# BjarkeHautop/bayesSSM

Measured on AMD Instinct MI355X. Metric: particle-steps/sec (N x T), bootstrap filter, higher is better.
Workload: dtype f64; 1 GPU; BASELINE C2: linear-Gaussian SSM, bootstrap filter, T=1000, N=1048576, SISR + systematic resampling, return_particles=FALSE, device generator; per_gpu=one independent filter replica per GPU (no data-path collective), backend=single process

## Files before the change

### bayesssm_amd/csrc/fused.hip.h

```cpp
#pragma once
#include "kernels.hip.h"

namespace bssm {

typedef unsigned long long fz_u64;
#define BSSM_RLX_AGENT __ATOMIC_RELAXED, __HIP_MEMORY_SCOPE_AGENT

constexpr int FZ_MAXB = 2 * NT;
constexpr int FZ_MINB = 256;
constexpr int FZ_KREC = 8;
constexpr int FZ_KSIDE = (int)(sizeof(SideEntry) / 4);
constexpr int FZ_NREP = 16;
constexpr int FZ_MAXSIDE = 16;
constexpr uint32_t FLAG_FUSED_BAIL = 8u, FLAG_FUSED_TIMEOUT = 16u;
constexpr uint32_t FZ_ST_DOIT = 1u, FZ_ST_DEAD = 2u, FZ_ST_STOP = 4u, FZ_ST_BAIL = 8u;
constexpr long long FZ_TIMEOUT_TICKS = 2000000ll;

struct FusedWs {
    fz_u64 e1[6][FZ_MAXB];
    fz_u64 c1[FZ_NREP][16];
    fz_u64 m1[FZ_NREP][16];
    fz_u64 a1[2][FZ_MAXB];
    fz_u64 e2[FZ_KREC][FZ_MAXB];
    fz_u64 c2[FZ_NREP][16];
    fz_u64 e3[FZ_KREC][FZ_MAXB];
    fz_u64 c3[FZ_NREP][16];
    fz_u64 a3[2][FZ_MAXB];
    fz_u64 side_w[FZ_MAXB][FZ_MAXSIDE][FZ_KSIDE];
    fz_u64 side_p[FZ_MAXB][FZ_MAXSIDE][FZ_KSIDE];
    BlockRec brec_priv[2][MAXB];
    SideList side_priv[2][FZ_MAXB];
    long long stamps[2][24];
    long long startt[FZ_MAXB];
    long long endt[FZ_MAXB];
    long long waket[4][FZ_MAXB];
    long long pubt[4][FZ_MAXB];
};

#ifdef BSSM_DEV_STAMPS
#define FZ_STAMP(k) do { if (fz_stamper) g.ws->stamps[fz_row][k] = clock64(); } while (0)
#else
#define FZ_STAMP(k) do { } while (0)
#endif

__device__ __forceinline__ fz_u64 fz_gran(uint32_t tag, uint32_t v) { return ((fz_u64)tag << 32) | v; }
__device__ __forceinline__ void fz_put(fz_u64* g, uint32_t tag, uint32_t v) { __hip_atomic_store(g, fz_gran(tag, v), BSSM_RLX_AGENT); }
__device__ __forceinline__ void fz_put64(fz_u64* g, uint32_t tag, uint64_t v) { fz_put(g, tag, (uint32_t)v); fz_put(g + 1, tag, (uint32_t)(v >> 32)); }
__device__ __forceinline__ void fz_put64x(fz_u64* g, int stride, uint32_t tag, uint64_t v) { fz_put(g, tag, (uint32_t)v); fz_put(g + stride, tag, (uint32_t)(v >> 32)); }
__device__ __forceinline__ fz_u64 fz_get(const fz_u64* g) { return __hip_atomic_load(g, BSSM_RLX_AGENT); }

__device__ __forceinline__ void fz_encode(const BlockRec& br, uint32_t (&w)[FZ_KREC])
{
    const Rec& r = br.prefix;
    const long long d1 = (long long)(r.o[1] - r.o[0]), d2 = (long long)(r.o[2] - r.o[0]), d3 = (long long)(r.o[3] - r.o[0]);
    const bool fits = d1 >= -32768 && d1 <= 32767 && d2 >= -32768 && d2 <= 32767 && d3 >= -32768 && d3 <= 32767;
    const uint32_t meta = (uint32_t)(r.kind & 3) | ((uint32_t)(br.nside & 127) << 2) | ((br.tail_from < NT) ? (1u << 9) : 0u) | (fits ? 0u : (1u << 10));
    w[0] = (uint32_t)r.base; w[1] = (uint32_t)(r.base >> 32); w[2] = (uint32_t)r.o[0]; w[3] = (uint32_t)(r.o[0] >> 32);
    w[4] = ((uint32_t)d1 & 0xffffu) | (((uint32_t)d2 & 0xffffu) << 16);
    w[5] = ((uint32_t)d3 & 0xffffu) | (meta << 16);
    w[6] = (uint32_t)r.lo; w[7] = (uint32_t)r.hi;
}
__device__ __forceinline__ BlockRec fz_decode(const uint32_t (&w)[FZ_KREC], bool& unsupported)
{
    BlockRec br;
    Rec& r = br.prefix;
    r.base = mk64(w[0], w[1]); r.o[0] = mk64(w[2], w[3]);
    r.o[1] = r.o[0] + (uint64_t)(long long)(int16_t)(w[4] & 0xffffu);
    r.o[2] = r.o[0] + (uint64_t)(long long)(int16_t)(w[4] >> 16);
    r.o[3] = r.o[0] + (uint64_t)(long long)(int16_t)(w[5] & 0xffffu);
    const uint32_t meta = w[5] >> 16;
    r.kind = (int32_t)(meta & 3); r.lo = (int32_t)w[6]; r.hi = (int32_t)w[7]; r.pad = 0;
    br.nside = (int32_t)((meta >> 2) & 127);
    const bool tail = (meta >> 9) & 1u, unenc = (meta >> 10) & 1u;
    br.tail_from = tail ? 0 : NT;
    unsupported = tail || unenc || br.nside > FZ_MAXSIDE;
    return br;
}

struct FzClock { long long t0; __device__ __forceinline__ bool expired() const { return (long long)wall_clock64() - t0 > FZ_TIMEOUT_TICKS; } };

template <int NG>
__device__ __forceinline__ bool fz_wait_slot(const fz_u64* slot, uint32_t tag, const FzClock& clk, uint32_t& val)
{
    const int lane = threadIdx.x & 63;
    for (unsigned spins = 0;; spins++) {
        bool ok = true;
        if (lane < NG) { const fz_u64 x = fz_get(slot + lane); ok = (uint32_t)(x >> 32) == tag; val = (uint32_t)x; }
        if (__all(ok)) return true;
        if ((spins & 31u) == 31u && clk.expired()) return false;
        __builtin_amdgcn_s_sleep(1);
    }
}

template <int NG>
__device__ __forceinline__ bool fz_wait_words(const fz_u64* mine, uint32_t tag, const FzClock& clk, uint32_t& val)
{
    const int lane = threadIdx.x & 63;
    for (unsigned spins = 0;; spins++) {
        bool ok = true;
        if (lane < NG) { const fz_u64 x = fz_get(mine); ok = (uint32_t)(x >> 32) == tag; val = (uint32_t)x; }
        if (__all(ok)) return true;
        if ((spins & 31u) == 31u && clk.expired()) return false;
        __builtin_amdgcn_s_sleep(1);
    }
}

struct LaneTerms { double a[EL]; };
__device__ __attribute__((noinline)) void fz_block_literal(uint64_t* tin , uint64_t cin, double* terms , const LaneTerms v ,
                                                           DevState* st)
{
    const int t = threadIdx.x;
#pragma unroll
    for (int k = 0; k < EL; k++) terms[t * EL + k] = v.a[k];
    __syncthreads();
    if (t == 0) {
        double c = b2d(cin);
        for (int tt = 0; tt < NT; tt++) {
            tin[tt] = d2b(c);
            for (int k = 0; k < EL; k++) c = c + terms[tt * EL + k];
        }
        atomicAdd((unsigned long long*)&st->stat_serial_walks, 1ull);
        atomicAdd((unsigned long long*)&st->stat_literal_terms, (unsigned long long)EB);
    }
    __syncthreads();
}
__device__ __forceinline__ LaneTerms fz_lane_terms(const double (&v)[EL])
{
    LaneTerms r;
#pragma unroll
    for (int k = 0; k < EL; k++) r.a[k] = v[k];
    return r;
}

struct FusedRecSink {
    fz_u64* rec_planes;
    fz_u64* side_base;
    int bidx; uint32_t tag;
    double* terms; DevState* st;
    __device__ __forceinline__ void rec(const BlockRec& br) const
    {
        uint32_t w[FZ_KREC];
        fz_encode(br, w);
#pragma unroll
        for (int k = 0; k < FZ_KREC; k++) fz_put(rec_planes + (size_t)k * FZ_MAXB + bidx, tag, w[k]);
    }
    __device__ __forceinline__ void side(int k, const SideEntry& e) const
    {
        if (k >= FZ_MAXSIDE) return;
        uint32_t w[FZ_KSIDE];
        memcpy(w, &e, sizeof(SideEntry));
        fz_u64* dst = side_base + ((size_t)bidx * FZ_MAXSIDE + k) * FZ_KSIDE;
#pragma unroll
        for (int q = 0; q < FZ_KSIDE; q++) fz_put(dst + q, tag, w[q]);
    }
    __device__ __forceinline__ void literal(uint64_t* tin, uint64_t cin, const double (&v)[EL]) const { fz_block_literal(tin, cin, terms, fz_lane_terms(v), st); }
};

struct FusedArgs {
    const double* xin;
    long long N; int nblk;
    ModelPar par; double y; NoiseSrc ns; int trans;
    int obs_i, resample_algorithm; double threshold;
    double* ess_out; double* llh_out; int* resampled_out;
    double* w_out;
    int lim;
    int force_fallback;
    int early_max;
    ApplyArgs a;
    FusedWs* ws; uint32_t tag;
    double* znext; uint32_t znext_call;
};

struct FusedSmem {
    double red[16]; double redq[16];
    uint32_t slot[16];
    int bail;
    double bm, bs_, bq;
};

template <int NG>
__device__ __forceinline__ bool fz_gather(const fz_u64* planes, int c0, int c1, uint32_t tag, const FzClock& clk, int* bail, uint32_t (&w0)[NG], uint32_t (&w1)[NG])
{
    const bool pair = ((c0 & 1) == 0) && (c0 < c1);
    const bool want1 = (c0 + 1 < c1);
    __amdgpu_buffer_rsrc_t rs = __builtin_amdgcn_make_buffer_rsrc((void*)const_cast<fz_u64*>(planes), 0, NG * FZ_MAXB * 8, 0x00020000);
    bool have = false;
    for (unsigned spins = 0;; spins++) {
        if (!have) {
            bool ok = true;
            if (pair) {
#pragma unroll
                for (int k = 0; k < NG; k++) {
                    const u32x4_t x = __builtin_amdgcn_raw_buffer_load_b128(rs, (k * FZ_MAXB + c0) * 8, 0, 16);
                    ok = ok && x.y == tag && (!want1 || x.w == tag); w0[k] = x.x; w1[k] = x.z;
                }
            } else {
#pragma unroll
                for (int k = 0; k < NG; k++) {
                    if (c0 < c1) { const fz_u64 x = fz_get(planes + (size_t)k * FZ_MAXB + c0); ok = ok && (uint32_t)(x >> 32) == tag; w0[k] = (uint32_t)x; }
                    if (c0 + 1 < c1) { const fz_u64 x = fz_get(planes + (size_t)k * FZ_MAXB + c0 + 1); ok = ok && (uint32_t)(x >> 32) == tag; w1[k] = (uint32_t)x; }
                }
            }
            have = ok;
        }
        if (__all(have)) return true;
        if ((spins & 15u) == 15u && clk.expired()) { *bail = 1; return false; }
        if (*(volatile int*)bail) return false;
        __builtin_amdgcn_s_sleep(1);
    }
}

__device__ __forceinline__ bool fz_fetch_sides(const fz_u64* side_base, SideList* side_priv, int b, int nside, uint32_t tag, const FzClock& clk)
{
    for (int k = 0; k < nside; k++) {
        const fz_u64* src = side_base + ((size_t)b * FZ_MAXSIDE + k) * FZ_KSIDE;
        uint32_t w[FZ_KSIDE];
        for (unsigned spins = 0;; spins++) {
            bool ok = true;
#pragma unroll
            for (int q = 0; q < FZ_KSIDE; q++) { const fz_u64 x = fz_get(src + q); ok = ok && (uint32_t)(x >> 32) == tag; w[q] = (uint32_t)x; }
            if (ok) break;
            if ((spins & 15u) == 15u && clk.expired()) return false;
            __builtin_amdgcn_s_sleep(1);
        }
        SideEntry e;
        memcpy(&e, w, sizeof(SideEntry));
        side_priv[b].e[k] = e;
    }
    return true;
}

struct FzLateSide {
    static constexpr bool active = true;
    const fz_u64* src; uint32_t tag; FzClock clk;
    __device__ __forceinline__ unsigned long long issue() const
    {
        const int lane = threadIdx.x & 63;
        static_assert(FZ_KSIDE <= 64, "one granule per lane");
        return (lane < FZ_KSIDE) ? fz_get(src + lane) : 0ull;
    }
    __device__ __forceinline__ bool finish(SideEntry* dst, unsigned long long x) const
    {
        const int lane = threadIdx.x & 63;
        for (unsigned spins = 0;; spins++) {
            const bool ok = (lane >= FZ_KSIDE) || ((uint32_t)(x >> 32) == tag);
            if (__all(ok)) {
                if (lane < FZ_KSIDE) reinterpret_cast<uint32_t*>(dst)[lane] = (uint32_t)x;
                __builtin_amdgcn_fence(__ATOMIC_RELEASE, "wavefront");
                __builtin_amdgcn_wave_barrier();
                __builtin_amdgcn_fence(__ATOMIC_ACQUIRE, "wavefront");
                return true;
            }
            if ((spins & 15u) == 15u && clk.expired()) return false;
            __builtin_amdgcn_s_sleep(1);
            if (lane < FZ_KSIDE) x = fz_get(src + lane);
        }
    }
};

template <int MODE, bool EMIT>
__device__ __forceinline__ uint64_t fz_resolve_duty(SegSmem& sm, ResolveSmem& rs, FusedSmem& fs, const FusedArgs& g, DevState* st, const FzClock& clk,
                                                    uint64_t* cin_lds , bool& bail)
{
    const int t = threadIdx.x, B = g.nblk;
    const fz_u64* planes = (MODE == MODE_W) ? &g.ws->e2[0][0] : &g.ws->e3[0][0];
    const fz_u64* sides = (MODE == MODE_W) ? &g.ws->side_w[0][0][0] : &g.ws->side_p[0][0][0];
    const int CB = (B + NT - 1) / NT;
    const int Bneed = (MODE == MODE_P) ? B - 1 : B;
    const int c0 = t * CB, c1 = (c0 + CB < Bneed) ? c0 + CB : Bneed;
    uint32_t w0[FZ_KREC], w1[FZ_KREC];
    bool ok = fz_gather<FZ_KREC>(planes, c0, c1, g.tag, clk, &fs.bail, w0, w1);
    bool unsup = false;
    BlockRec q0, q1;
    q0.prefix = rec_identity(0); q0.tail_from = NT; q0.nside = 0; q1 = q0;
    if (ok) {
        if (c0 < c1) {
            bool u; q0 = fz_decode(w0, u); unsup = unsup || u;
            if (!u && q0.nside > 0 && !(c0 == B - 1 && q0.nside == 1 && q0.tail_from >= NT)) {
#ifdef BSSM_DEV_STAMPS
                g.ws->pubt[3][20 + MODE] = c0; atomicAdd((unsigned long long*)&g.ws->pubt[3][22 + MODE], 1ull);
#endif
                ok = ok && fz_fetch_sides(sides, g.ws->side_priv[MODE], c0, q0.nside, g.tag, clk);
            }
        }
        if (c0 + 1 < c1) {
            bool u; q1 = fz_decode(w1, u); unsup = unsup || u;
            if (!u && q1.nside > 0 && !(c0 + 1 == B - 1 && q1.nside == 1 && q1.tail_from >= NT)) {
#ifdef BSSM_DEV_STAMPS
                g.ws->pubt[3][20 + MODE] = c0 + 1; atomicAdd((unsigned long long*)&g.ws->pubt[3][22 + MODE], 1ull);
#endif
                ok = ok && fz_fetch_sides(sides, g.ws->side_priv[MODE], c0 + 1, q1.nside, g.tag, clk);
            }
        }
    }
    if (unsup) atomicMax(&fs.bail, 2); else if (!ok) atomicMax(&fs.bail, 1);
    __syncthreads();
#ifdef BSSM_DEV_STAMPS
    if (t == 0) { g.ws->stamps[1][MODE == MODE_W ? 8 : 13] = clock64(); g.ws->pubt[3][8 + (MODE == MODE_W ? 1 : 2)] = (long long)wall_clock64(); }
#endif
    if (fs.bail) { bail = true; return 0ull; }
    long long lit = 0;
    const int upto = (MODE == MODE_P) ? B - 1 : B;
    FzLateSide late; late.src = sides + ((size_t)(B - 1) * FZ_MAXSIDE + 0) * FZ_KSIDE; late.tag = g.tag; late.clk = clk;
    const uint64_t fin = resolve_in_block<MODE, NT, EMIT, FzLateSide>(sm, rs, g.ws->brec_priv[MODE], g.ws->side_priv[MODE], B, upto, g.xin, g.N, 1.0, st, true, g.force_fallback, cin_lds, &lit, &q0, &q1, late);
    if (EMIT && t == 0) cin_lds[B - 1] = fin;
    if (lit >= LIT_FROM_W) fs.bail = 2;
    __syncthreads();
#ifdef BSSM_DEV_STAMPS
    if (t == 0) g.ws->stamps[1][MODE == MODE_W ? 9 : 14] = clock64();
#endif
    if (fs.bail) { bail = true; return 0ull; }
    return fin;
}

__host__ __device__ __forceinline__ int fz_resolver_block(int B) { return (5 * B) / 16; }

__device__ __forceinline__ void fz_draw_next(const FusedArgs& g, long long j0, long long N, const int prio_after = 1)
{
    if (!g.znext) return;
    __builtin_amdgcn_s_setprio(0);
#pragma unroll
    for (int i = 0; i < EL / 2; i++) {
        const long long j = j0 + 2 * i;
        if (j < N) {
            double z0, z1;
            normal_pair(g.ns.key, g.ns.purpose, g.znext_call, 0, (uint32_t)(j >> 1), z0, z1);
            if (j + 1 < N) bulk_store16<1>(g.znext + j, z0, z1);
            else g.znext[j] = z0;
        }
    }
    if (prio_after == 3) __builtin_amdgcn_s_setprio(3); else __builtin_amdgcn_s_setprio(1);
}

template <int MODEL, int KIND>
__global__ __launch_bounds__(NT) void k_obs(FusedArgs g, DevState* st)
{
    __shared__ SegSmem sm;
    __shared__ uint64_t tin[NT + 1];
    __shared__ FusedSmem fs;
    __shared__ int Tbegin;
    extern __shared__ __attribute__((aligned(16))) double dyn[];
    int* Tl = reinterpret_cast<int*>(dyn);
    double* lx = dyn + EB / 2;
    const int t = threadIdx.x, lane = t & 63, wave = t >> 6;
    const int bidx = (int)blockIdx.x, B = g.nblk;
    const bool resolver = (bidx == fz_resolver_block(B));
    if (resolver) __builtin_amdgcn_s_setprio(3); else __builtin_amdgcn_s_setprio(1);
    const bool fz_stamper = (t == 0) && (resolver || bidx == ((B > 100) ? 100 : 0)); const int fz_row = resolver ? 1 : 0; (void)fz_stamper; (void)fz_row;
    FZ_STAMP(0);
#ifdef BSSM_DEV_STAMPS
    if (t == 0) g.ws->startt[bidx] = (long long)wall_clock64();
#define FZ_PUBT(k) do { if (t == 0) g.ws->pubt[k][bidx] = (long long)wall_clock64(); } while (0)
#define FZ_GDONE(k) do { if (t == 0) g.ws->pubt[3][8 + (k)] = (long long)wall_clock64(); } while (0)
#define FZ_WAKE(k) do { if (t == 0) g.ws->waket[k][bidx] = (long long)wall_clock64(); } while (0)
#else
#define FZ_PUBT(k) do { } while (0)
#define FZ_GDONE(k) do { } while (0)
#define FZ_WAKE(k) do { } while (0)
#endif
    const long long b0 = (long long)bidx * EB, j0 = b0 + (long long)t * EL;
    const long long N = g.N;
    FzClock clk; clk.t0 = (long long)wall_clock64();
    const int s_dead = st->dead, call = st->res_calls;
    const uint32_t s_flags = st->flags;
    if (t == 0) fs.bail = 0;
    double x8[EL], l8[EL];
    if (j0 + EL <= N) {
        const double2* p = reinterpret_cast<const double2*>(g.xin + j0);
#pragma unroll
        for (int k = 0; k < EL / 2; k++) { const double2 q = p[k]; x8[2 * k] = q.x; x8[2 * k + 1] = q.y; }
    } else {
#pragma unroll
        for (int k = 0; k < EL; k++) x8[k] = (j0 + k < N) ? g.xin[j0 + k] : 0.0;
    }
    double z8[EL];
#pragma unroll
    for (int i = 0; i < EL / 2; i++) {
        const long long j = j0 + 2 * i;
        z8[2 * i] = 0.0; z8[2 * i + 1] = 0.0;
        if (g.trans && j < N) {
            if (g.ns.arr) { if (j + 1 < N) { const double2 q = *reinterpret_cast<const double2*>(g.ns.arr + j); z8[2 * i] = q.x; z8[2 * i + 1] = q.y; } else { z8[2 * i] = g.ns.arr[j]; } }
            else normal_pair(g.ns.key, g.ns.purpose, g.ns.call, 0, (uint32_t)(j >> 1), z8[2 * i], z8[2 * i + 1]);
        }
    }
    if (s_dead || s_flags) return;
#pragma unroll
    for (int i = 0; i < EL / 2; i++) {
        const long long j = j0 + 2 * i;
        if (g.trans && j < N) {
            x8[2 * i] = Model<MODEL>::transition(x8[2 * i], z8[2 * i], g.par);
            x8[2 * i + 1] = Model<MODEL>::transition(x8[2 * i + 1], z8[2 * i + 1], g.par);
        }
        l8[2 * i] = (j < N) ? r_dnorm_log(g.y, x8[2 * i], g.par.sy, g.par.log_sy) : -INFINITY;
        l8[2 * i + 1] = (j + 1 < N) ? r_dnorm_log(g.y, x8[2 * i + 1], g.par.sy, g.par.log_sy) : -INFINITY;
    }
    FZ_STAMP(1);
    double bm;
    {
        double m = l8[0];
#pragma unroll
        for (int k = 1; k < EL; k++) m = fmax(m, l8[k]);
        m = wave_max(m);
        __syncthreads();
        if (lane == 0) fs.red[wave] = m;
        __syncthreads();
        bm = fs.red[0];
#pragma unroll
        for (int i = 1; i < NWV; i++) bm = fmax(bm, fs.red[i]);
    }
    const bool early = (g.early_max != 0);
    if (early && t < 2) { const uint64_t bits = d2b(bm); fz_put(&g.ws->e1[t][bidx], g.tag, t ? (uint32_t)(bits >> 32) : (uint32_t)bits); }
    double bsum, bsq;
    {
        double sv[EL / 2], qv[EL / 2];
#pragma unroll
        for (int i = 0; i < EL / 2; i++) {
            double s_ = 0.0, q_ = 0.0;
            if (bm > -INFINITY) {
                if (l8[2 * i] > -INFINITY) { const double e = exp_nonpos(l8[2 * i] - bm); s_ += e; q_ += e * e; }
                if (l8[2 * i + 1] > -INFINITY) { const double e = exp_nonpos(l8[2 * i + 1] - bm); s_ += e; q_ += e * e; }
            }
            sv[i] = s_; qv[i] = q_;
        }
        static_assert(EL == 8, "four k_step pairs per lane");
        double s4 = (sv[0] + sv[1]) + (sv[2] + sv[3]), q4 = (qv[0] + qv[1]) + (qv[2] + qv[3]);
#define STEP(C) s4 = dpp_f64<C, 0xf>(0.0, s4) + s4; q4 = dpp_f64<C, 0xf>(0.0, q4) + q4;
        STEP(DPP_SHR1) STEP(DPP_SHR2) STEP(DPP_SHR4) STEP(DPP_SHR8)
#undef STEP
        __syncthreads();
        if ((lane & 15) == 15) { fs.red[4 * wave + (lane >> 4)] = s4; fs.redq[4 * wave + (lane >> 4)] = q4; }
        __syncthreads();
        double s_ = 0.0, q_ = 0.0;
#pragma unroll
        for (int i = 0; i < 16; i++) { s_ += fs.red[i]; q_ += fs.redq[i]; }
        bsum = s_; bsq = q_;
    }
    if (t < 6 && !(early && t < 2)) {
        const uint64_t bits = d2b(t < 2 ? bm : (t < 4 ? bsum : bsq));
        fz_put(&g.ws->e1[t][bidx], g.tag, (t & 1) ? (uint32_t)(bits >> 32) : (uint32_t)bits);
    }
    FZ_STAMP(2); FZ_PUBT(0);
    if (resolver) {
        const int L = (B + NT - 1) / NT;
        const int c0 = t * L, c1 = (c0 + L < B) ? c0 + L : B;
        uint32_t status = 0;
        double M = 0.0, S = 0.0, sq = 0.0, ess1 = 0.0;
        double pmv[2] = {-INFINITY, -INFINITY}, psv[2] = {0.0, 0.0}, pqv[2] = {0.0, 0.0}, exv[2] = {0.0, 0.0};
        if (early) {
            uint32_t a0[2], a1[2];
            if (!fz_gather<2>(&g.ws->e1[0][0], c0, c1, g.tag, clk, &fs.bail, a0, a1)) fs.bail = 1;
            __syncthreads();
            const bool bail1 = (fs.bail != 0);
            if (!bail1) {
                if (c0 < c1) pmv[0] = b2d(mk64(a0[0], a0[1]));
                if (c0 + 1 < c1) pmv[1] = b2d(mk64(a1[0], a1[1]));
                M = block_max(fmax(pmv[0], pmv[1]), sm.sh4);
            }
            if (t < FZ_NREP) fz_put64(&g.ws->m1[t][0], g.tag, d2b(M));
            FZ_GDONE(3);
            if (!bail1) {
#pragma unroll
                for (int k = 0; k < 2; k++) if (pmv[k] > -INFINITY) exv[k] = exp_nonpos(pmv[k] - M);
                uint32_t s0[4], s1[4];
                if (!fz_gather<4>(&g.ws->e1[2][0], c0, c1, g.tag, clk, &fs.bail, s0, s1)) fs.bail = 1;
                if (c0 < c1) { psv[0] = b2d(mk64(s0[0], s0[1])); pqv[0] = b2d(mk64(s0[2], s0[3])); }
                if (c0 + 1 < c1) { psv[1] = b2d(mk64(s1[0], s1[1])); pqv[1] = b2d(mk64(s1[2], s1[3])); }
            }
            __syncthreads();
        } else {
            uint32_t w0[6], w1[6];
            if (!fz_gather<6>(&g.ws->e1[0][0], c0, c1, g.tag, clk, &fs.bail, w0, w1)) fs.bail = 1;
            __syncthreads();
            if (!fs.bail) {
                if (c0 < c1) { pmv[0] = b2d(mk64(w0[0], w0[1])); psv[0] = b2d(mk64(w0[2], w0[3])); pqv[0] = b2d(mk64(w0[4], w0[5])); }
                if (c0 + 1 < c1) { pmv[1] = b2d(mk64(w1[0], w1[1])); psv[1] = b2d(mk64(w1[2], w1[3])); pqv[1] = b2d(mk64(w1[4], w1[5])); }
                M = block_max(fmax(pmv[0], pmv[1]), sm.sh4);
            }
        }
        FZ_STAMP(3); FZ_GDONE(0);
        bool book = false;
        double esv[2] = {0.0, 0.0}, pre = 0.0;
        if (!fs.bail) {
            const bool degenerate = (M < -1e8);
            if (degenerate) {
                if (t == 0) { st->loglike = -INFINITY; g.llh_out[g.obs_i - 1] = -INFINITY; st->dead = g.obs_i; st->do_resample = 0; }
                status = FZ_ST_DEAD;
            } else {
                double ts0 = 0.0, tq = 0.0;
#pragma unroll
                for (int k = 0; k < 2; k++) {
                    double x = 0.0;
                    if (pmv[k] > -INFINITY) { const double ex = early ? exv[k] : exp_nonpos(pmv[k] - M); x = psv[k] * ex; tq += pqv[k] * ex * ex; }
                    esv[k] = x; ts0 += x;
                }
                const double inc = wave_incl_sum(ts0);
                const double exc = dpp_f64<DPP_WAVE_SHR1, 0xf>(0.0, inc);
                const double wq = wave_sum(tq);
                __syncthreads();
                if (lane == 63) { sm.sh4[wave] = inc; sm.sh4[8 + wave] = wq; }
                __syncthreads();
                pre = exc;
                for (int i = 0; i < wave; i++) pre += sm.sh4[i];
                S = tree_sum<NWV>(sm.sh4);
                sq = tree_sum<NWV>(sm.sh4 + 8);
                ess1 = 1.0 / (sq / (S * S));
                const int doit = (g.resample_algorithm == 0) ? 0 : (g.resample_algorithm == 1) ? 1 : (ess1 < g.threshold);
                book = true;
                status = doit ? FZ_ST_DOIT : 0u;
                if (doit && (!(S > 0.0) || !isfinite(S) || !isfinite(M))) {
                    if (t == 0) atomicOr(&st->flags, FLAG_NONFINITE);
                    status |= FZ_ST_STOP;
                }
            }
        } else {
            status = FZ_ST_BAIL;
            if (t == 0) atomicOr(&st->flags, FLAG_FUSED_TIMEOUT);
        }
        {
            double pp = pre;
#pragma unroll
            for (int k = 0; k < 2; k++) {
                const int i = c0 + k;
                if (k < L && i < c1) fz_put64x(&g.ws->a1[0][i], FZ_MAXB, g.tag, d2b(pp / S));
                pp += esv[k];
            }
            if (t < FZ_NREP) {
                fz_u64* rep = &g.ws->c1[t][0];
                fz_put64(rep + 0, g.tag, d2b(M)); fz_put64(rep + 2, g.tag, d2b(S)); fz_put64(rep + 4, g.tag, d2b(sq)); fz_put(rep + 6, g.tag, status);
            }
        }
        if (book && t == 0) {
            const int doit = (status & FZ_ST_DOIT) ? 1 : 0;
            const double ll = st->loglike + (M + log(S) - log((double)N));
            st->loglike = ll; g.llh_out[g.obs_i - 1] = ll;
            st->do_resample = doit;
            g.ess_out[g.obs_i] = doit ? (double)N : ess1;
            if (g.resampled_out) g.resampled_out[g.obs_i - 1] = doit;
            st->ess = ess1; st->lse_max = M; st->lse_sum = S;
            if (doit) { st->cur_call = call; st->res_calls = call + 1; }
        }
    }
    if (resolver) FZ_STAMP(4);
    double v[EL];
    if (early) {
        if (wave == 0) {
            uint32_t vv = 0;
            const bool ok = fz_wait_slot<2>(&g.ws->m1[bidx % FZ_NREP][0], g.tag, clk, vv);
            if (lane < 2) fs.slot[10 + lane] = vv;
            if (!ok && lane == 0) fs.bail = 1;
        }
        __syncthreads();
        if (fs.bail) { if (t == 0 && fs.bail == 1) atomicOr(&st->flags, FLAG_FUSED_TIMEOUT); return; }
        const double Me = b2d(mk64(fs.slot[10], fs.slot[11]));
        FZ_STAMP(19); FZ_WAKE(3);
#pragma unroll
        for (int k = 0; k < EL; k++) v[k] = (j0 + k < N) ? exp_nonpos(l8[k] - Me) : 0.0;
    }
    double M, S, a_in;
    uint32_t status;
    {
        if (wave == 0) {
            uint32_t v = 0;
            const fz_u64* src = (lane < 7) ? &g.ws->c1[bidx % FZ_NREP][lane] : &g.ws->a1[(lane - 7) & 1][bidx];
            const bool ok = fz_wait_words<9>(src, g.tag, clk, v);
            if (lane < 9) fs.slot[lane] = v;
            if (!ok && lane == 0) fs.bail = 1;
        }
        __syncthreads();
        if (fs.bail) { if (t == 0 && fs.bail == 1) atomicOr(&st->flags, FLAG_FUSED_TIMEOUT); return; }
        M = b2d(mk64(fs.slot[0], fs.slot[1])); S = b2d(mk64(fs.slot[2], fs.slot[3])); a_in = b2d(mk64(fs.slot[7], fs.slot[8]));
        status = fs.slot[6];
    }
    FZ_STAMP(5); FZ_WAKE(0);
    if (status & (FZ_ST_DEAD | FZ_ST_BAIL)) return;
    const bool doit = status & FZ_ST_DOIT;
    if (early) {
#pragma unroll
        for (int k = 0; k < EL; k++) v[k] = (j0 + k < N) ? v[k] / S : 0.0;
    } else {
#pragma unroll
        for (int k = 0; k < EL; k++) v[k] = (j0 + k < N) ? exp_nonpos(l8[k] - M) / S : 0.0;
    }
    if (g.w_out) {
        if (j0 + EL <= N) {
#pragma unroll
            for (int k = 0; k < EL / 2; k++) bulk_store16<BSSM_ST_W>(g.w_out + j0 + 2 * k, v[2 * k], v[2 * k + 1]);
        } else {
#pragma unroll
            for (int k = 0; k < EL; k++) if (j0 + k < N) g.w_out[j0 + k] = v[k];
        }
    }
    if (!doit) {
        double* xa = lx; double* wa = lx + EB;
        __syncthreads();
#pragma unroll
        for (int k = 0; k < EL; k++) { xa[t * EL + k] = x8[k]; wa[t * EL + k] = v[k]; }
        __syncthreads();
        double acc0 = 0.0;
#pragma unroll
        for (int r = 0; r < EL; r++) {
            const long long j = b0 + t + NT * r;
            if (j < N) { const double x0 = xa[t + NT * r]; g.a.xdst[j] = x0; acc0 += x0 * wa[t + NT * r]; }
        }
        acc0 = block_sum(acc0, sm.sh4);
        if (t == 0) g.a.se_part[bidx] = acc0;
        fz_draw_next(g, j0, N);
        return;
    }
    if (status & FZ_ST_STOP) return;
    FZ_STAMP(6);
    FusedRecSink sink; sink.bidx = bidx; sink.tag = g.tag; sink.terms = lx; sink.st = st;
    {
        BlockScan bsw;
        block_scan<MODE_W>(sm, v, a_in, g.lim, bsw);
        __syncthreads();
        sink.rec_planes = &g.ws->e2[0][0]; sink.side_base = &g.ws->side_w[0][0][0];
        block_record_tail<MODE_W, 11>(sm, tin, bsw, v, a_in, g.lim, st, 0, false, sink);
    }
    FZ_STAMP(7); FZ_PUBT(1);
    if (!resolver) fz_draw_next(g, j0, N);
    ResolveSmem& rs = *reinterpret_cast<ResolveSmem*>(dyn);
    uint64_t* cin_lds = reinterpret_cast<uint64_t*>(reinterpret_cast<char*>(dyn) + ((sizeof(ResolveSmem) + 15) / 16) * 16);
    if (resolver) {
        __syncthreads();
        bool bail = false;
        const uint64_t fin = fz_resolve_duty<MODE_W, false>(sm, rs, fs, g, st, clk, nullptr, bail);
        uint32_t stw = 0;
        if (bail) { stw = FZ_ST_BAIL; if (t == 0) atomicOr(&st->flags, fs.bail == 1 ? FLAG_FUSED_TIMEOUT : FLAG_FUSED_BAIL); }
        else {
            const double tot = b2d(fin);
            if (t == 0) {
                st->total_bits = fin;
                if (tot == 0.0) atomicOr(&st->flags, FLAG_ZERO_SUM);
                if (!isfinite(tot)) atomicOr(&st->flags, FLAG_NONFINITE);
            }
            if (tot == 0.0 || !isfinite(tot)) stw = FZ_ST_STOP;
        }
        if (t < FZ_NREP) { fz_put64(&g.ws->c2[t][0], g.tag, fin); fz_put(&g.ws->c2[t][2], g.tag, stw); }
        fz_draw_next(g, j0, N);
        FZ_STAMP(10);
    }
    double total;
    {
        __syncthreads();
        if (wave == 0) {
            uint32_t vv = 0;
            const bool ok = fz_wait_slot<3>(&g.ws->c2[bidx % FZ_NREP][0], g.tag, clk, vv);
            if (lane < 3) fs.slot[lane] = vv;
            if (!ok && lane == 0) fs.bail = 1;
        }
        __syncthreads();
        if (fs.bail) { if (t == 0 && fs.bail == 1) atomicOr(&st->flags, FLAG_FUSED_TIMEOUT); return; }
        if (fs.slot[2] & (FZ_ST_BAIL | FZ_ST_STOP)) return;
        total = b2d(mk64(fs.slot[0], fs.slot[1]));
    }
    FZ_STAMP(11); FZ_WAKE(1);
    const double a_in_p = a_in / total;
#pragma unroll
    for (int k = 0; k < EL; k++) v[k] = v[k] / total;
    BlockScan bs;
#ifdef BSSM_DEV_STAMPS
    const bool xstamper = (t == 0 && bidx == B / 4);
    const int xdbg = 99;
    if (xstamper) st->stamps[2][10] = clock64();
#else
    const bool xstamper = false; const int xdbg = 0;
#endif
    block_scan<MODE_P>(sm, v, a_in_p, g.lim, bs);
    __syncthreads();
#ifdef BSSM_DEV_STAMPS
    if (xstamper) st->stamps[2][11] = clock64();
#endif
    sink.rec_planes = &g.ws->e3[0][0]; sink.side_base = &g.ws->side_p[0][0][0];
    block_record_tail<MODE_P, 3>(sm, tin, bs, v, a_in_p, g.lim, st, xdbg, xstamper, sink);
#ifdef BSSM_DEV_STAMPS
    if (xstamper) { st->stamps[2][9] = clock64(); st->stamps[2][8] = bs.nb; }
#endif
    FZ_STAMP(12); FZ_PUBT(2);
    uint64_t cinb = 0;
    if (resolver) {
        __syncthreads();
        bool bail = false;
        (void)fz_resolve_duty<MODE_P, true>(sm, rs, fs, g, st, clk, cin_lds, bail);
        uint32_t stp = 0;
        if (bail) { stp = FZ_ST_BAIL; if (t == 0) atomicOr(&st->flags, fs.bail == 1 ? FLAG_FUSED_TIMEOUT : FLAG_FUSED_BAIL); }
        for (int b = t; b < B; b += NT) fz_put64x(&g.ws->a3[0][b], FZ_MAXB, g.tag, bail ? 0ull : cin_lds[b]);
        if (t < FZ_NREP) fz_put(&g.ws->c3[t][0], g.tag, stp);
        FZ_STAMP(15);
        if (bail) return;
        cinb = cin_lds[bidx];
        __syncthreads();
    } else {
        __syncthreads();
        if (wave == 0) {
            uint32_t vv = 0;
            const fz_u64* src = (lane < 2) ? &g.ws->a3[lane & 1][bidx] : &g.ws->c3[bidx % FZ_NREP][0];
            const bool ok = fz_wait_words<3>(src, g.tag, clk, vv);
            if (lane < 3) fs.slot[lane] = vv;
            if (!ok && lane == 0) fs.bail = 1;
        }
        __syncthreads();
        if (fs.bail) { if (t == 0 && fs.bail == 1) atomicOr(&st->flags, FLAG_FUSED_TIMEOUT); return; }
        if (fs.slot[2] & FZ_ST_BAIL) return;
        cinb = mk64(fs.slot[0], fs.slot[1]);
    }
    FZ_STAMP(16); FZ_WAKE(2);
    uint64_t ent;
    {
        const bool good = block_resolve<MODE_P>(sm, bs, cinb, g.lim, nullptr, 0, total, b0, ent);
        if (!good) { fz_block_literal(tin, cinb, lx, fz_lane_terms(v), st); ent = tin[t]; }
    }
    FZ_STAMP(17);
    double xs0[EL], xs1[EL], axs[EL];
    __syncthreads();
#pragma unroll
    for (int k = 0; k < EL; k++) lx[t * EL + k] = x8[k];
    __syncthreads();
    {
        const int ebase = wave * (64 * EL) + lane;
#pragma unroll
        for (int k = 0; k < EL; k++) { xs0[k] = lx[ebase + 64 * k]; xs1[k] = 0.0; axs[k] = 0.0; }
    }
    if (t == 0) sm.big = 0;
    UniformSrc us;
    us.arr = g.a.u_base ? g.a.u_base + (long long)call * g.a.u_stride : nullptr;
    us.key = g.a.key; us.call = (uint32_t)call;
    const double Usys = (KIND == 1) ? us(0) : 0.0;
    __syncthreads();
    apply_tail<KIND, false, CAPX, false>(sm, Tl, Tbegin, bidx, B, g.a, st, g.a.nstage ? lx + EB : nullptr, g.a.nstage, v, ent, xs0, xs1, axs, call, us, Usys, 0, false, lx);
    FZ_STAMP(18);
#ifdef BSSM_DEV_STAMPS
    if (t == 0) g.ws->pubt[3][32 + (bidx & 255)] = 0;
    __syncthreads();
    if (t == 0) g.ws->endt[bidx] = (long long)wall_clock64();
#endif
}

constexpr size_t FZ_DYN_LDS = (size_t)EB * sizeof(int) + (size_t)(EB + CAPX) * sizeof(double);
static_assert(((sizeof(ResolveSmem) + 15) / 16) * 16 + FZ_MAXB * sizeof(uint64_t) <= FZ_DYN_LDS, "the resolver's scratch borrows the workers' staging area");

}
```

Baseline: 22.56 billion particle-steps/s.

## Publish early sum separately and let resolver skip self-waits in fused obs kernel

In the early path of the fused observation kernel, the resolver publishes the weight sum S to a dedicated replicated slot (s1) right after its reduction. Other blocks can then normalise weights as soon as S arrives instead of waiting for the full c1 record. The resolver block fills its own shared-memory slots locally and no longer polls global flags it wrote itself, and its bookkeeping writes (loglike, ESS, outputs) are deferred off the critical path. Block 0 also skips waiting on its prefix word. The cost is an extra set of global flag writes and more complex branching, with some risk of ordering errors in the deferred bookkeeping.

New measurement: 23.06 billion particle-steps/s (median of 6 runs). 2.2% higher.

```diff
diff --git a/bayesssm_amd/csrc/fused.hip.h b/bayesssm_amd/csrc/fused.hip.h
--- a/bayesssm_amd/csrc/fused.hip.h
+++ b/bayesssm_amd/csrc/fused.hip.h
@@ -20,6 +20,7 @@
     fz_u64 e1[6][FZ_MAXB];
     fz_u64 c1[FZ_NREP][16];
     fz_u64 m1[FZ_NREP][16];
+    fz_u64 s1[FZ_NREP][16];
     fz_u64 a1[2][FZ_MAXB];
     fz_u64 e2[FZ_KREC][FZ_MAXB];
     fz_u64 c2[FZ_NREP][16];
@@ -33,7 +34,7 @@
     long long stamps[2][24];
     long long startt[FZ_MAXB];
     long long endt[FZ_MAXB];
-    long long waket[4][FZ_MAXB];
+    long long waket[5][FZ_MAXB];
     long long pubt[4][FZ_MAXB];
 };
 
@@ -175,7 +176,7 @@
     double red[16]; double redq[16];
     uint32_t slot[16];
     int bail;
-    double bm, bs_, bq;
+    int book; double ess1;
 };
 
 template <int NG>
@@ -332,6 +333,18 @@
     if (prio_after == 3) __builtin_amdgcn_s_setprio(3); else __builtin_amdgcn_s_setprio(1);
 }
 
+__device__ __forceinline__ void fz_book(const FusedArgs& g, DevState* st, long long N, int call, double M, double S, double ess1, uint32_t status)
+{
+    const int doit = (status & FZ_ST_DOIT) ? 1 : 0;
+    const double ll = st->loglike + (M + log(S) - log((double)N));
+    st->loglike = ll; g.llh_out[g.obs_i - 1] = ll;
+    st->do_resample = doit;
+    g.ess_out[g.obs_i] = doit ? (double)N : ess1;
+    if (g.resampled_out) g.resampled_out[g.obs_i - 1] = doit;
+    st->ess = ess1; st->lse_max = M; st->lse_sum = S;
+    if (doit) { st->cur_call = call; st->res_calls = call + 1; }
+}
+
 template <int MODEL, int KIND>
 __global__ __launch_bounds__(NT) void k_obs(FusedArgs g, DevState* st)
 {
@@ -363,7 +376,7 @@
     FzClock clk; clk.t0 = (long long)wall_clock64();
     const int s_dead = st->dead, call = st->res_calls;
     const uint32_t s_flags = st->flags;
-    if (t == 0) fs.bail = 0;
+    if (t == 0) { fs.bail = 0; fs.book = 0; }
     double x8[EL], l8[EL];
     if (j0 + EL <= N) {
         const double2* p = reinterpret_cast<const double2*>(g.xin + j0);
@@ -478,7 +491,7 @@
             }
         }
         FZ_STAMP(3); FZ_GDONE(0);
-        bool book = false;
+        bool book = false, s_sent = false;
         double esv[2] = {0.0, 0.0}, pre = 0.0;
         if (!fs.bail) {
             const bool degenerate = (M < -1e8);
@@ -502,6 +515,7 @@
                 pre = exc;
                 for (int i = 0; i < wave; i++) pre += sm.sh4[i];
                 S = tree_sum<NWV>(sm.sh4);
+                if (early) { if (t < FZ_NREP) fz_put64(&g.ws->s1[t][0], g.tag, d2b(S)); s_sent = true; FZ_GDONE(4); }
                 sq = tree_sum<NWV>(sm.sh4 + 8);
                 ess1 = 1.0 / (sq / (S * S));
                 const int doit = (g.resample_algorithm == 0) ? 0 : (g.resample_algorithm == 1) ? 1 : (ess1 < g.threshold);
@@ -517,33 +531,39 @@
             if (t == 0) atomicOr(&st->flags, FLAG_FUSED_TIMEOUT);
         }
         {
+            if (early && !s_sent && t < FZ_NREP) fz_put64(&g.ws->s1[t][0], g.tag, d2b(S));
             double pp = pre;
 #pragma unroll
             for (int k = 0; k < 2; k++) {
                 const int i = c0 + k;
-                if (k < L && i < c1) fz_put64x(&g.ws->a1[0][i], FZ_MAXB, g.tag, d2b(pp / S));
+                if (k < L && i < c1) {
+                    const uint64_t abits = d2b(pp / S);
+                    fz_put64x(&g.ws->a1[0][i], FZ_MAXB, g.tag, abits);
+                    if (early && i == bidx) { fs.slot[7] = (uint32_t)abits; fs.slot[8] = (uint32_t)(abits >> 32); }
+                }
                 pp += esv[k];
             }
             if (t < FZ_NREP) {
                 fz_u64* rep = &g.ws->c1[t][0];
                 fz_put64(rep + 0, g.tag, d2b(M)); fz_put64(rep + 2, g.tag, d2b(S)); fz_put64(rep + 4, g.tag, d2b(sq)); fz_put(rep + 6, g.tag, status);
             }
+            if (early && t == 0) {
+                const uint64_t mb = d2b(M), sb = d2b(S), qb = d2b(sq);
+                fs.slot[0] = (uint32_t)mb; fs.slot[1] = (uint32_t)(mb >> 32); fs.slot[2] = (uint32_t)sb; fs.slot[3] = (uint32_t)(sb >> 32);
+                fs.slot[4] = (uint32_t)qb; fs.slot[5] = (uint32_t)(qb >> 32); fs.slot[6] = status;
+                fs.slot[10] = (uint32_t)mb; fs.slot[11] = (uint32_t)(mb >> 32); fs.slot[12] = (uint32_t)sb; fs.slot[13] = (uint32_t)(sb >> 32);
+            }
         }
         if (book && t == 0) {
-            const int doit = (status & FZ_ST_DOIT) ? 1 : 0;
-            const double ll = st->loglike + (M + log(S) - log((double)N));
-            st->loglike = ll; g.llh_out[g.obs_i - 1] = ll;
-            st->do_resample = doit;
-            g.ess_out[g.obs_i] = doit ? (double)N : ess1;
-            if (g.resampled_out) g.resampled_out[g.obs_i - 1] = doit;
-            st->ess = ess1; st->lse_max = M; st->lse_sum = S;
-            if (doit) { st->cur_call = call; st->res_calls = call + 1; }
+            if (early) { fs.book = 1; fs.ess1 = ess1; }
+            else fz_book(g, st, N, call, M, S, ess1, status);
         }
     }
     if (resolver) FZ_STAMP(4);
     double v[EL];
+    const bool own = early && resolver;
     if (early) {
-        if (wave == 0) {
+        if (!own && wave == 0) {
             uint32_t vv = 0;
             const bool ok = fz_wait_slot<2>(&g.ws->m1[bidx % FZ_NREP][0], g.tag, clk, vv);
             if (lane < 2) fs.slot[10 + lane] = vv;
@@ -555,28 +575,45 @@
         FZ_STAMP(19); FZ_WAKE(3);
 #pragma unroll
         for (int k = 0; k < EL; k++) v[k] = (j0 + k < N) ? exp_nonpos(l8[k] - Me) : 0.0;
+        if (!own) {
+            if (wave == 0) {
+                uint32_t vv = 0;
+                const bool ok = fz_wait_slot<2>(&g.ws->s1[bidx % FZ_NREP][0], g.tag, clk, vv);
+                if (lane < 2) fs.slot[12 + lane] = vv;
+                if (!ok && lane == 0) fs.bail = 1;
+            }
+            __syncthreads();
+            if (fs.bail) { if (t == 0 && fs.bail == 1) atomicOr(&st->flags, FLAG_FUSED_TIMEOUT); return; }
+        }
+        const double Se = b2d(mk64(fs.slot[12], fs.slot[13]));
+        FZ_STAMP(20); FZ_WAKE(4);
+#pragma unroll
+        for (int k = 0; k < EL; k++) v[k] = (j0 + k < N) ? v[k] / Se : 0.0;
     }
     double M, S, a_in;
     uint32_t status;
     {
-        if (wave == 0) {
-            uint32_t v = 0;
-            const fz_u64* src = (lane < 7) ? &g.ws->c1[bidx % FZ_NREP][lane] : &g.ws->a1[(lane - 7) & 1][bidx];
-            const bool ok = fz_wait_words<9>(src, g.tag, clk, v);
-            if (lane < 9) fs.slot[lane] = v;
-            if (!ok && lane == 0) fs.bail = 1;
-        }
-        __syncthreads();
-        if (fs.bail) { if (t == 0 && fs.bail == 1) atomicOr(&st->flags, FLAG_FUSED_TIMEOUT); return; }
-        M = b2d(mk64(fs.slot[0], fs.slot[1])); S = b2d(mk64(fs.slot[2], fs.slot[3])); a_in = b2d(mk64(fs.slot[7], fs.slot[8]));
+        const bool head = early && bidx == 0;
+        if (!own) {
+            if (wave == 0) {
+                uint32_t v = 0;
+                const fz_u64* src = (lane < 7) ? &g.ws->c1[bidx % FZ_NREP][lane] : &g.ws->a1[(lane - 7) & 1][bidx];
+                const bool ok = head ? fz_wait_words<7>(src, g.tag, clk, v) : fz_wait_words<9>(src, g.tag, clk, v);
+                if (lane < (head ? 7 : 9)) fs.slot[lane] = v;
+                if (!ok && lane == 0) fs.bail = 1;
+            }
+            __syncthreads();
+            if (fs.bail) { if (t == 0 && fs.bail == 1) atomicOr(&st->flags, FLAG_FUSED_TIMEOUT); return; }
+        }
+        M = b2d(mk64(fs.slot[0], fs.slot[1])); S = b2d(mk64(fs.slot[2], fs.slot[3]));
+        a_in = (head && !own) ? 0.0 : b2d(mk64(fs.slot[7], fs.slot[8]));
         status = fs.slot[6];
     }
     FZ_STAMP(5); FZ_WAKE(0);
     if (status & (FZ_ST_DEAD | FZ_ST_BAIL)) return;
     const bool doit = status & FZ_ST_DOIT;
+    auto book_late = [&]() { if (own && t == 0 && fs.book) fz_book(g, st, N, call, M, S, fs.ess1, status); };
     if (early) {
-#pragma unroll
-        for (int k = 0; k < EL; k++) v[k] = (j0 + k < N) ? v[k] / S : 0.0;
     } else {
 #pragma unroll
         for (int k = 0; k < EL; k++) v[k] = (j0 + k < N) ? exp_nonpos(l8[k] - M) / S : 0.0;
@@ -604,10 +641,11 @@
         }
         acc0 = block_sum(acc0, sm.sh4);
         if (t == 0) g.a.se_part[bidx] = acc0;
+        book_late();
         fz_draw_next(g, j0, N);
         return;
     }
-    if (status & FZ_ST_STOP) return;
+    if (status & FZ_ST_STOP) { book_late(); return; }
     FZ_STAMP(6);
     FusedRecSink sink; sink.bidx = bidx; sink.tag = g.tag; sink.terms = lx; sink.st = st;
     {
@@ -618,6 +656,7 @@
         block_record_tail<MODE_W, 11>(sm, tin, bsw, v, a_in, g.lim, st, 0, false, sink);
     }
     FZ_STAMP(7); FZ_PUBT(1);
+    book_late();
     if (!resolver) fz_draw_next(g, j0, N);
     ResolveSmem& rs = *reinterpret_cast<ResolveSmem*>(dyn);
     uint64_t* cin_lds = reinterpret_cast<uint64_t*>(reinterpret_cast<char*>(dyn) + ((sizeof(ResolveSmem) + 15) / 16) * 16);
@@ -637,13 +676,14 @@
             if (tot == 0.0 || !isfinite(tot)) stw = FZ_ST_STOP;
         }
         if (t < FZ_NREP) { fz_put64(&g.ws->c2[t][0], g.tag, fin); fz_put(&g.ws->c2[t][2], g.tag, stw); }
+        if (own && t == 0) { fs.slot[0] = (uint32_t)fin; fs.slot[1] = (uint32_t)(fin >> 32); fs.slot[2] = stw; }
         fz_draw_next(g, j0, N);
         FZ_STAMP(10);
     }
     double total;
     {
         __syncthreads();
-        if (wave == 0) {
+        if (!own && wave == 0) {
             uint32_t vv = 0;
             const bool ok = fz_wait_slot<3>(&g.ws->c2[bidx % FZ_NREP][0], g.tag, clk, vv);
             if (lane < 3) fs.slot[lane] = vv;
```
